# jerry102102102/RL_brain_trainer

Measured on NVIDIA B200. Metric: kinematic_env_steps_per_sec_policy_in_loop, higher is better.
Workload: dtype f32 env + f16 MLP operands (f32 accumulate)

## Files before the change

rl_brain_trainer_b200/csrc/kin_rollout_tc16.cu:

```cuda
#include <cstdlib>

#include "kin_tc16.cuh"

namespace kin {

using namespace tc16;

#ifdef KIN_TC16_TRACE
__device__ long long kin_tc16_trace_buf[8][16][12];
#define TC16_STAMP(slot) do { if (blockIdx.x == 0 && c.step_id >= 10 && c.step_id < 18 && (threadIdx.x & 31) == 0) \
        kin_tc16_trace_buf[c.step_id - 10][threadIdx.x >> 5][slot] = clock64(); } while (0)
#else
#define TC16_STAMP(slot)
#endif

struct Tile16 {
    unsigned char *X, *H;
    float* snap;
    unsigned x_lo, h_lo, w0_lo, w1_lo, wo_lo, wob_lo;
    unsigned mbar_saddr, cnt_saddr, full_saddr, tmem_d, tmem_row;
    unsigned x_row, h_row;
    volatile int* stamp;
    int row, n_warps;
    unsigned parity, arrivals;
    int step_id;
};

template <bool AT>
__device__ __forceinline__ void issue_layer16(int layer, unsigned tmem_d, unsigned x_lo, unsigned h_lo, unsigned w0_lo, unsigned w1_lo,
                                              unsigned wo_lo, unsigned wob_lo, unsigned mbar_saddr) {
    auto mma = [&](unsigned a, int ka, unsigned b_lo, unsigned id, unsigned acc) {
        if constexpr (AT) mma_f16_ts(tmem_d, a + 8u * ka, b_lo, id, acc);
        else mma_f16(tmem_d, a + 2u * ka, b_lo, id, acc);
    };
    if (layer == 0) {
        constexpr unsigned id = idesc_f16(TILE, HID);
#pragma unroll
        for (int k = 0; k < X_K / 16; ++k) mma(x_lo, k, w0_lo + 2 * k, id, k > 0 ? 1u : 0u);
    } else if (layer == 1) {
        constexpr unsigned id = idesc_f16(TILE, HID);
#pragma unroll
        for (int k = 0; k < HID / 16; ++k) mma(h_lo, k, w1_lo + 2 * k, id, k > 0 ? 1u : 0u);
        mma(x_lo, 2, w0_lo + 6, id, 1u);
    } else {
        constexpr unsigned id = idesc_f16(TILE, 16);
#pragma unroll
        for (int k = 0; k < HID / 16; ++k) mma(h_lo, k, wo_lo + 2 * k, id, k > 0 ? 1u : 0u);
        mma(x_lo, 2, wob_lo + 4, id, 1u);
    }
    umma::commit(mbar_saddr);
}

template <bool ISS, bool AT>
__device__ __forceinline__ void tile_sync16(Tile16& c, int layer, int sid) {
    TC16_STAMP(layer);
    if constexpr (AT) tmem_st_wait();
    if constexpr (ISS) {
        if constexpr (!AT) umma::fence_async_smem();
        umma::fence_before();
        __syncwarp();
        if ((threadIdx.x & 31) == 0) mbar_arrive(c.full_saddr);
    } else {
        c.arrivals += (unsigned)c.n_warps;
        if (const int last = tile_arrive(c.cnt_saddr, c.arrivals, layer == 0 ? c.stamp : nullptr, sid)) {
            umma::fence_after();
            if (elect_one()) {
                if (last == 1) issue_layer16<AT>(layer, c.tmem_d, c.x_lo, c.h_lo, c.w0_lo, c.w1_lo, c.wo_lo, c.wob_lo, c.mbar_saddr);
                else mbar_arrive(c.mbar_saddr);
            }
            __syncwarp();
            TC16_STAMP(6 + layer);
        }
    }
    mbar_wait_or_trap(c.mbar_saddr, c.parity);
    TC16_STAMP(3 + layer);
    c.parity ^= 1u;
}

template <bool ISS, bool AT>
__device__ __forceinline__ bool mlp16(Tile16& c, const unsigned* w, float* act, bool running) {
    const int sid = ++c.step_id;
    if (__any_sync(0xffffffffu, running) && (threadIdx.x & 31) == 0) *c.stamp = sid;
    if constexpr (AT) {
        tmem_st8(c.x_row, w);
        tmem_st8(c.x_row + 8u, w + 8);
        tmem_st4(c.x_row + 16u, w[16], w[17], 0x00003C00u, 0u);
    } else {
        st_chunk(c.X, c.row, 0, w[0], w[1], w[2], w[3]);
        st_chunk(c.X, c.row, 1, w[4], w[5], w[6], w[7]);
        st_chunk(c.X, c.row, 2, w[8], w[9], w[10], w[11]);
        st_chunk(c.X, c.row, 3, w[12], w[13], w[14], w[15]);
        st_chunk(c.X, c.row, 4, w[16], w[17], 0x00003C00u, 0u);
    }
    tile_sync16<ISS, AT>(c, 0, sid);
    if (*c.stamp != sid) return false;
    umma::fence_after();
    if constexpr (AT) epilogue_tanh_tmem(c.tmem_row, c.h_row);
    else epilogue_tanh(c.tmem_row, c.H, c.row);
    tile_sync16<ISS, AT>(c, 1, sid);
    umma::fence_after();
    if constexpr (AT) epilogue_tanh_tmem(c.tmem_row, c.h_row);
    else epilogue_tanh(c.tmem_row, c.H, c.row);
    tile_sync16<ISS, AT>(c, 2, sid);
    umma::fence_after();
    {
        float o[8];
        tmem_ld8(c.tmem_row, o);
#pragma unroll
        for (int i = 0; i < NJ; ++i) act[i] = clampf(o[i], -1.0f, 1.0f);
    }
    return true;
}

struct IssTile {
    unsigned x_lo, h_lo, tmem_d, full_saddr, mbar_saddr;
    volatile int* stamp;
    unsigned parity;
    int sid, layer, tile;
    bool exists, live;
};

template <bool AT>
__device__ __forceinline__ void issuer_poll(IssTile& t, unsigned w0_lo, unsigned w1_lo, unsigned wo_lo, unsigned wob_lo, unsigned hint_ns) {
    if (!(hint_ns ? mbar_try_wait_hint(t.full_saddr, t.parity, hint_ns) : mbar_test_wait(t.full_saddr, t.parity))) return;
    t.parity ^= 1u;
    umma::fence_after();
    bool go = true;
    if (t.layer == 0) {
        t.sid += 1;
        go = (*t.stamp == t.sid);
    }
#ifdef KIN_TC16_TRACE
    if (blockIdx.x == 0 && t.sid >= 10 && t.sid < 18 && (threadIdx.x & 31) == 0) kin_tc16_trace_buf[t.sid - 10][4 * t.tile][9 + t.layer] = clock64();
#endif
    if (elect_one()) {
        if (go) issue_layer16<AT>(t.layer, t.tmem_d, t.x_lo, t.h_lo, w0_lo, w1_lo, wo_lo, wob_lo, t.mbar_saddr);
        else mbar_arrive(t.mbar_saddr);
#ifdef KIN_TC16_TRACE
        if (blockIdx.x == 0 && t.sid >= 10 && t.sid < 18) kin_tc16_trace_buf[t.sid - 10][4 * t.tile][6 + t.layer] = clock64();
#endif
    }
    __syncwarp();
    if (!go) t.live = false;
    else t.layer = t.layer == 2 ? 0 : t.layer + 1;
}

__device__ unsigned kin_tc16_poll_hint = 32u;

template <bool AT>
__device__ __forceinline__ void issuer_phase(IssTile& a, IssTile& b, unsigned w0_lo, unsigned w1_lo, unsigned wo_lo, unsigned wob_lo) {
    a.live = a.exists;
    b.live = b.exists;
    a.layer = b.layer = 0;
    unsigned spins = 0u;
    while (a.live || b.live) {
        const unsigned hint = (a.live && b.live) ? kin_tc16_poll_hint : 1000u;
        if (a.live) issuer_poll<AT>(a, w0_lo, w1_lo, wo_lo, wob_lo, hint);
        if (b.live) issuer_poll<AT>(b, w0_lo, w1_lo, wo_lo, wob_lo, hint);
        if (++spins > (1u << 28)) __trap();
    }
}

__device__ __forceinline__ bool ready_pred16(float pos_thr, float ori_thr, float a_thr, float dq_thr, float pos, float ori, float an, float dqn) {
    return pos_thr > 0.0f && ori_thr > 0.0f && pos <= pos_thr && ori <= ori_thr && (a_thr <= 0.0f || an <= a_thr) && (dq_thr <= 0.0f || dqn <= dq_thr);
}

template <int FAST, bool ISS, bool AT>
__global__ void __launch_bounds__(MAX_THREADS, 1)
kin_rollout_tc16_kernel(const __grid_constant__ KinEnvParams PA, const __grid_constant__ KinEnvParams PF, DevPolicy pol_a, DevPolicy pol_f,
                        int has_finisher, const float* __restrict__ iq, const float* __restrict__ idq, const float* __restrict__ ipa,
                        const float* __restrict__ gq, const float* __restrict__ gpose, int n, int stride, int confirm,
                        uint32_t* __restrict__ result, unsigned long long* __restrict__ env_steps) {
    extern __shared__ __align__(1024) unsigned char smem_raw[];
    unsigned char* base = smem_raw + ((1024u - (umma::smem_u32(smem_raw) & 1023u)) & 1023u);
    Smem& S = *reinterpret_cast<Smem*>(base);
    const int tid = threadIdx.x;
    const int warp = tid >> 5;
    const int env_threads = (int)blockDim.x - (ISS ? 64 : 0);
    const int n_tiles_cta = (env_threads + TILE - 1) / TILE;
    unsigned char* tiles = base + ((sizeof(Smem) + 1023) / 1024) * 1024;
    float* snaps = reinterpret_cast<float*>(tiles + (size_t)n_tiles_cta * 2 * TILE_BYTES);

    Tile16 c;
    const int tile = tid >> 7;
    c.row = tid & (TILE - 1);
    c.n_warps = (min(TILE, env_threads - tile * TILE) + 31) >> 5;
    c.X = tiles + (size_t)tile * 2 * TILE_BYTES;
    c.H = c.X + TILE_BYTES;
    c.snap = snaps + (size_t)tile * SNAP_FLOATS * TILE + c.row;
    c.parity = 0u;
    c.arrivals = 0u;
    c.step_id = 0;
    c.stamp = &S.run_stamp[tile];

    constexpr unsigned TCOLS = AT ? 128u : 64u;
    const unsigned tmem_cols = n_tiles_cta == 1 ? TCOLS : (n_tiles_cta == 2 ? 2u * TCOLS : 4u * TCOLS);
    if (warp == 0) umma::tmem_alloc(umma::smem_u32(&S.tmem_base), tmem_cols);
    if (tid == 0) {
#pragma unroll
        for (int i = 0; i < MAX_TILES; ++i) {
            umma::mbar_init(umma::smem_u32(&S.mbar[i]), 1);
            umma::mbar_init(umma::smem_u32(&S.full[i]), (unsigned)max(1, (min(TILE, env_threads - i * TILE) + 31) >> 5));
            S.arrive[i] = 0u;
            S.run_stamp[i] = 0;
        }
        umma::fence_mbar_init();
    }
    load_weights(S, pol_a, KIN_MODE_APPROACH, tid, (int)blockDim.x);
    const bool env_thread = tid < env_threads;
    if (env_thread) {
#pragma unroll
        for (int ch = 0; ch < 8; ++ch) {
            st_chunk(c.X, c.row, ch, 0u, 0u, 0u, 0u);
            st_chunk(c.H, c.row, ch, 0u, 0u, 0u, 0u);
        }
    }
    if (env_thread && c.n_warps < 4) {
        for (int r = c.n_warps * 32 + c.row; r < TILE; r += c.n_warps * 32)
#pragma unroll
            for (int ch = 0; ch < 8; ++ch) {
                st_chunk(c.X, r, ch, 0u, 0u, 0u, 0u);
                st_chunk(c.H, r, ch, 0u, 0u, 0u, 0u);
            }
    }
    umma::fence_async_smem();
    umma::fence_before();
    __syncthreads();
    umma::fence_after();
    const unsigned tmem_base = S.tmem_base;
    c.x_lo = desc_lo(umma::smem_u32(c.X));
    c.h_lo = desc_lo(umma::smem_u32(c.H));
    c.w0_lo = desc_lo(umma::smem_u32(S.W0));
    c.w1_lo = desc_lo(umma::smem_u32(S.W1));
    c.wo_lo = desc_lo(umma::smem_u32(S.WO));
    c.wob_lo = desc_lo(umma::smem_u32(S.WOB));
    c.mbar_saddr = umma::smem_u32(&S.mbar[tile]);
    c.cnt_saddr = umma::smem_u32(&S.arrive[tile]);
    c.full_saddr = umma::smem_u32(&S.full[tile]);
    c.tmem_d = tmem_base + tile * TCOLS;
    c.tmem_row = c.tmem_d + ((unsigned)((warp & 3) * 32) << 16);
    c.h_row = c.tmem_row + 64u;
    c.x_row = c.tmem_row + 96u;
    if constexpr (AT) {
        c.x_lo = c.tmem_d + 96u;
        c.h_lo = c.tmem_d + 64u;
        if (env_thread) {
            tmem_st4(c.x_row + 20u, 0u, 0u, 0u, 0u);
            tmem_st4(c.x_row + 24u, 0u, 0u, 0u, 0u);
            tmem_st4(c.x_row + 28u, 0u, 0u, 0u, 0u);
            tmem_st_wait();
        }
    }

    if constexpr (ISS) {
        if (!env_thread) {
            const int iw = (tid - env_threads) >> 5;
            IssTile it[2];
#pragma unroll
            for (int j = 0; j < 2; ++j) {
                const int t = 2 * iw + j;
                it[j].exists = t < n_tiles_cta;
                it[j].tile = t;
                unsigned char* X = tiles + (size_t)t * 2 * TILE_BYTES;
                it[j].x_lo = desc_lo(umma::smem_u32(X));
                it[j].h_lo = desc_lo(umma::smem_u32(X + TILE_BYTES));
                it[j].tmem_d = tmem_base + t * TCOLS;
                if constexpr (AT) { it[j].x_lo = it[j].tmem_d + 96u; it[j].h_lo = it[j].tmem_d + 64u; }
                it[j].full_saddr = umma::smem_u32(&S.full[t]);
                it[j].mbar_saddr = umma::smem_u32(&S.mbar[t]);
                it[j].stamp = &S.run_stamp[t];
                it[j].parity = 0u;
                it[j].sid = 0;
            }
            issuer_phase<AT>(it[0], it[1], c.w0_lo, c.w1_lo, c.wo_lo, c.wob_lo);
            __syncthreads();
            if (has_finisher) {
                load_weights(S, pol_f, KIN_MODE_DOCK, tid, (int)blockDim.x);
                umma::fence_async_smem();
                __syncthreads();
                issuer_phase<AT>(it[0], it[1], c.w0_lo, c.w1_lo, c.wo_lo, c.wob_lo);
            }
            umma::fence_before();
            __syncthreads();
            return;
        }
    }

    const int ep = blockIdx.x * env_threads + tid;
    const bool active = ep < n;
    const int epc = active ? ep : n - 1;

    EnvRegs s;
    s.flags = 0u;
    float goal_q[NJ];
    {
        float r_iq[NJ], r_idq[NJ], r_ipa[NJ], r_gq[NJ], r_gp[6];
#pragma unroll
        for (int k = 0; k < NJ; ++k) {
            r_iq[k] = iq[(size_t)epc * NJ + k];
            r_idq[k] = idq ? idq[(size_t)epc * NJ + k] : 0.0f;
            r_ipa[k] = ipa ? ipa[(size_t)epc * NJ + k] : 0.0f;
            r_gq[k] = gq ? gq[(size_t)epc * NJ + k] : 0.0f;
        }
        if (gpose) {
#pragma unroll
            for (int k = 0; k < 6; ++k) r_gp[k] = gpose[(size_t)epc * 6 + k];
        }
        reset_core(PA, s, KIN_MODE_APPROACH, r_iq, r_idq, r_ipa, r_gq, gpose ? r_gp : nullptr, goal_q);
    }

    float min_pos = s.entry[0], min_ori = s.entry[1];
    int steps = 0, streak = 0, max_streak = 0, first_ready = -1;
    bool ready_hit = false, have_snap = false;
    int snap_step = -1;
    float last_an = 0.0f, last_dqn = 0.0f;
    StepOut so;
    prime_step_out(PA, s, so);
    bool running = active;
    while (true) {
        unsigned w[X_DYN / 2];
        float act[NJ];
        obs_pack(PA, s, so, w);
        if (!mlp16<ISS, AT>(c, w, act, running)) break;
        if (running) {
            step_core<KIN_MODE_APPROACH, false, FAST>(PA, s, act, so, nullptr);
            const float an = so.action_l2;
            steps += 1;
            min_pos = fminf(min_pos, so.pos);
            min_ori = fminf(min_ori, so.ori);
            if (ready_pred16(PA.ar_dock_coarse_ready_pos_threshold_m, PA.ar_dock_coarse_ready_ori_threshold_rad,
                             PA.ar_dock_coarse_ready_action_threshold, PA.ar_dock_coarse_ready_dq_threshold, so.pos, so.ori, an, so.dq_l2)) {
                ready_hit = true;
                if (first_ready < 0) first_ready = steps;
                streak += 1;
            } else {
                streak = 0;
            }
            max_streak = max(max_streak, streak);
            if (!have_snap && streak >= confirm) {
                have_snap = true;
                snap_step = steps;
#pragma unroll
                for (int i = 0; i < NJ; ++i) {
                    c.snap[i * TILE] = s.q[i];
                    c.snap[(NJ + i) * TILE] = s.dq[i];
                    c.snap[(2 * NJ + i) * TILE] = s.pa[i];
                }
            }
            last_an = an;
            last_dqn = so.dq_l2;
            running = !(so.done & (KIN_DONE_TERMINATED | KIN_DONE_TRUNCATED));
        }
    }
    if (active) {
        result[(size_t)KIN_RES_APPROACH_ACTION * stride + ep] = __float_as_uint(last_an);
        result[(size_t)KIN_RES_APPROACH_DQ * stride + ep] = __float_as_uint(last_dqn);
    }
    const int approach_steps = steps;
    const bool approach_success = (so.done & KIN_DONE_SUCCESS) != 0;
    const float approach_pos = so.pos, approach_ori = so.ori;
    const bool final_ready = ready_pred16(PA.ar_finisher_ready_pos_threshold_m, PA.ar_finisher_ready_ori_threshold_rad,
                                          PA.ar_finisher_ready_action_threshold, PA.ar_finisher_ready_dq_threshold, so.pos, so.ori, last_an, last_dqn);
    const int handoff_kind = final_ready ? 2 : (have_snap ? 1 : 0);
    const int handoff_step = final_ready ? steps : (have_snap ? snap_step : -1);
    bool success = approach_success;
    float final_pos = so.pos, final_ori = so.ori, final_an = last_an, final_dqn = last_dqn;
    int finisher_steps = 0;

    __syncthreads();
    if (has_finisher) {
        load_weights(S, pol_f, KIN_MODE_DOCK, tid, (int)blockDim.x);
        umma::fence_async_smem();
        __syncthreads();
        running = active && handoff_kind != 0;
        if (running) {
            float r_iq[NJ], r_idq[NJ], r_ipa[NJ], gq_out[NJ], r_gp[6];
#pragma unroll
            for (int i = 0; i < NJ; ++i) {
                r_iq[i] = (handoff_kind == 2) ? s.q[i] : c.snap[i * TILE];
                r_idq[i] = (handoff_kind == 2) ? s.dq[i] : c.snap[(NJ + i) * TILE];
                r_ipa[i] = (handoff_kind == 2) ? s.pa[i] : c.snap[(2 * NJ + i) * TILE];
            }
#pragma unroll
            for (int k = 0; k < 6; ++k) r_gp[k] = s.goal[k];
            reset_core(PF, s, KIN_MODE_DOCK, r_iq, r_idq, r_ipa, goal_q, r_gp, gq_out);
        }
        steps = 0;
        prime_step_out(PF, s, so);
        if (!running) { so.pos = final_pos; so.ori = final_ori; }
        while (true) {
            unsigned w[X_DYN / 2];
            float act[NJ];
            obs_pack(PF, s, so, w);
            if (!mlp16<ISS, AT>(c, w, act, running)) break;
            if (running) {
                float an2 = 0.0f;
#pragma unroll
                for (int i = 0; i < NJ; ++i) an2 = fmaf(act[i], act[i], an2);
                step_core<KIN_MODE_DOCK, false, FAST>(PF, s, act, so, nullptr);
                steps += 1;
                final_an = sqrt_approx(an2);
                running = !(so.done & (KIN_DONE_TERMINATED | KIN_DONE_TRUNCATED));
            }
        }
        if (active && handoff_kind != 0) {
            finisher_steps = steps;
            success = (so.done & KIN_DONE_SUCCESS) != 0;
            final_pos = so.pos; final_ori = so.ori; final_dqn = so.dq_l2;
        }
    }

    if (active) {
        auto put_u = [&](int row, uint32_t v) { result[(size_t)row * stride + ep] = v; };
        auto put_f = [&](int row, float v) { result[(size_t)row * stride + ep] = __float_as_uint(v); };
        put_u(KIN_RES_SUCCESS, success ? 1u : 0u);
        put_u(KIN_RES_FLAGS, (approach_success ? 1u : 0u) | ((ready_hit || final_ready) ? 2u : 0u) |
                                 ((max_streak >= confirm || final_ready) ? 4u : 0u) | (final_ready ? 8u : 0u) | ((uint32_t)handoff_kind << 4));
        put_u(KIN_RES_HANDOFF_STEP, (uint32_t)handoff_step);
        put_u(KIN_RES_FIRST_READY_STEP, (uint32_t)first_ready);
        put_u(KIN_RES_MAX_READY_STREAK, (uint32_t)max_streak);
        put_u(KIN_RES_STEPS, (uint32_t)approach_steps | ((uint32_t)finisher_steps << 16));
        put_f(KIN_RES_FINAL_POS, final_pos); put_f(KIN_RES_FINAL_ORI, final_ori);
        put_f(KIN_RES_APPROACH_POS, approach_pos); put_f(KIN_RES_APPROACH_ORI, approach_ori);
        put_f(KIN_RES_MIN_POS, min_pos); put_f(KIN_RES_MIN_ORI, min_ori);
        put_f(KIN_RES_FINAL_ACTION, final_an); put_f(KIN_RES_FINAL_DQ, final_dqn);
#pragma unroll
        for (int i = 0; i < NJ; ++i) put_f(KIN_RES_FINAL_Q + i, s.q[i]);
    }
    if (env_steps) {
        unsigned long long mine = active ? (unsigned long long)(approach_steps + finisher_steps) : 0ull;
#pragma unroll
        for (int off = 16; off > 0; off >>= 1) mine += __shfl_xor_sync(0xffffffffu, mine, off);
        if ((tid & 31) == 0 && mine) atomicAdd(env_steps, mine);
    }
    umma::fence_before();
    __syncthreads();
    if (warp == 0) umma::tmem_dealloc(tmem_base, tmem_cols);
}

}

using namespace kin;

#ifdef KIN_TC16_TRACE
extern "C" int kin_debug_tc16_trace(long long* out) {
    return cudaMemcpyFromSymbol(out, kin_tc16_trace_buf, sizeof(kin_tc16_trace_buf)) == cudaSuccess ? KIN_OK : KIN_ERR_INVALID_ARG;
}
#endif

int kin_rollout_tc16_launch(const KinHandle* ha, const KinHandle* hf, const KinPolicyWeights* pa, const KinPolicyWeights* pf,
                            const float* iq, const float* idq, const float* ipa, const float* gq, const float* gpose, int n, int stride,
                            int confirm, uint32_t* result, unsigned long long* env_steps, cudaStream_t st) {
    using Kernel = void (*)(KinEnvParams, KinEnvParams, tc16::DevPolicy, tc16::DevPolicy, int, const float*, const float*, const float*, const float*,
                            const float*, int, int, int, uint32_t*, unsigned long long*);
    static const Kernel kernels[2][2][2] = {{{kin_rollout_tc16_kernel<1, false, false>, kin_rollout_tc16_kernel<1, false, true>},
                                             {kin_rollout_tc16_kernel<1, true, false>, kin_rollout_tc16_kernel<1, true, true>}},
                                            {{kin_rollout_tc16_kernel<2, false, false>, kin_rollout_tc16_kernel<2, false, true>},
                                             {kin_rollout_tc16_kernel<2, true, false>, kin_rollout_tc16_kernel<2, true, true>}}};
    static bool attr_set[KIN_MAX_DEVICES] = {};
    const int dev_slot = kin_device_slot();
    if (!attr_set[dev_slot]) {
        for (int i = 0; i < 8; ++i) {
            cudaError_t e = cudaFuncSetAttribute(kernels[i >> 2][(i >> 1) & 1][i & 1], cudaFuncAttributeMaxDynamicSharedMemorySize, (int)tc16::smem_bytes(tc16::MAX_TILES));
            if (e != cudaSuccess) return kin_fail_cuda(e, "kin_rollout_approach_finisher(tc16): smem attribute");
        }
        attr_set[dev_slot] = true;
    }
    static const bool exact_sincos = kin_env_flag("KIN_TC16_EXACT_SINCOS");
    static const bool no_issuer = kin_env_flag("KIN_TC16_NO_ISSUER_WARPS");
    static const bool tmem_a = !kin_env_flag("KIN_TC16_SMEM_A");
    static bool hint_set = false;
    if (!hint_set) {
        if (const char* v = getenv("KIN_TC16_POLL_HINT")) { const unsigned h = (unsigned)atoi(v); cudaMemcpyToSymbol(kin_tc16_poll_hint, &h, sizeof(h)); }
        hint_set = true;
    }
    tc16::DevPolicy da{pa->pi_w0, pa->pi_b0, pa->pi_w1, pa->pi_b1, pa->act_w, pa->act_b};
    tc16::DevPolicy df = pf ? tc16::DevPolicy{pf->pi_w0, pf->pi_b0, pf->pi_w1, pf->pi_b1, pf->act_w, pf->act_b} : da;
    const KinEnvParams& PF = hf ? hf->params : ha->params;
    static int n_sm = 0;
    if (n_sm == 0) {
        int dev = 0;
        if (cudaGetDevice(&dev) != cudaSuccess || cudaDeviceGetAttribute(&n_sm, cudaDevAttrMultiProcessorCount, dev) != cudaSuccess || n_sm <= 0) n_sm = 148;
    }
    const int warps = (n + 31) / 32;
    int w_per_cta = (warps + n_sm - 1) / n_sm;
    if (w_per_cta > 16) w_per_cta = 16;
    if (const char* v = getenv("KIN_TC_WARPS")) { const int f = atoi(v); if (f >= 1 && f <= 16) w_per_cta = f; }
    const bool iss = w_per_cta <= 14 && !no_issuer;
    const int env_threads = 32 * w_per_cta;
    const int threads = env_threads + (iss ? 64 : 0);
    const size_t smem = tc16::smem_bytes((env_threads + tc16::TILE - 1) / tc16::TILE);
    kernels[exact_sincos ? 0 : 1][iss ? 1 : 0][tmem_a ? 1 : 0]<<<(n + env_threads - 1) / env_threads, threads, smem, st>>>(
        ha->params, PF, da, df, (hf && pf) ? 1 : 0, iq, idq, ipa, gq, gpose, n, stride, confirm, result, env_steps);
    cudaError_t e = cudaGetLastError();
    return e == cudaSuccess ? KIN_OK : kin_fail_cuda(e, "kin_rollout_approach_finisher(tc16)");
}
```

rl_brain_trainer_b200/csrc/kin_tc16.cuh:

```cuda
#pragma once

#include <cuda_fp16.h>

#include "kin_internal.h"
#include "kin_state.cuh"
#include "kin_umma.cuh"

namespace kin {
namespace tc16 {

using namespace umma;

constexpr int TILE = 128;
constexpr int MAX_TILES = 4;
constexpr int MAX_THREADS = TILE * MAX_TILES;
constexpr int HID = 64;
constexpr int X_DYN = 36;
constexpr int X_ONE = 36;
constexpr int X_K = 48;
constexpr int B1_COL = 52;
constexpr int TILE_BYTES = TILE * 128;
constexpr int SNAP_FLOATS = 3 * KIN_NJ;

struct Smem {
    alignas(1024) unsigned char W0[HID * 128];
    alignas(1024) unsigned char W1[HID * 128];
    alignas(1024) unsigned char WO[16 * 128];
    alignas(1024) unsigned char WOB[16 * 128];
    unsigned long long mbar[MAX_TILES];
    unsigned long long full[MAX_TILES];
    unsigned arrive[MAX_TILES];
    int run_stamp[MAX_TILES];
    unsigned tmem_base;
};

struct DevPolicy {
    const float *w0, *b0, *w1, *b1, *wo, *bo;
};

__host__ __device__ constexpr size_t smem_bytes(int n_tiles) {
    return ((sizeof(Smem) + 1023) / 1024) * 1024 + (size_t)n_tiles * (2 * TILE_BYTES + SNAP_FLOATS * TILE * sizeof(float)) + 1024;
}

__host__ __device__ constexpr unsigned idesc_f16(int M, int N) { return (1u << 4) | ((unsigned)(N >> 3) << 17) | ((unsigned)(M >> 4) << 24); }

__device__ __forceinline__ unsigned pack_h2(float lo, float hi) {
    unsigned r;
    asm("cvt.rn.f16x2.f32 %0, %1, %2;" : "=r"(r) : "f"(hi), "f"(lo));
    return r;
}
__device__ __forceinline__ unsigned clamp1_h2(unsigned x) {
    unsigned y;
    asm("{\n\t.reg .b32 t;\n\tmax.f16x2 t, %1, %2;\n\tmin.f16x2 %0, t, %3;\n\t}" : "=r"(y) : "r"(x), "r"(0xBC00BC00u), "r"(0x3C003C00u));
    return y;
}
__device__ __forceinline__ void st_chunk(unsigned char* img, int row, int chunk, unsigned a, unsigned b, unsigned c, unsigned d) {
    *reinterpret_cast<uint4*>(img + umma::sw_chunk(row, chunk)) = make_uint4(a, b, c, d);
}

__device__ __forceinline__ int dyn_col(int k) { return k < 20 ? k : (k < 27 ? k + 10 : (k < 29 ? k + 10 : k + 11)); }

__device__ __forceinline__ void obs_pack(const KinEnvParams& P, const EnvRegs& s, const StepOut& so, unsigned* w) {
    float v[X_DYN];
#pragma unroll
    for (int i = 0; i < NJ; ++i) {
        v[i] = s.dq[i] * P.k_inv_delta_limit[i];
        v[13 + i] = so.margin[i];
        v[20 + i] = s.pa[i];
        v[29 + i] = so.qn[i];
    }
#pragma unroll
    for (int k = 0; k < 3; ++k) {
        v[7 + k] = so.oe[k] * P.k_inv_ori_err_scale;
        v[10 + k] = so.pe[k] * P.k_inv_pos_err_scale;
    }
    v[27] = (float)s.step * P.k_inv_episode_length;
    v[28] = (float)s.dwell * P.k_inv_dwell_steps_target;
#pragma unroll
    for (int i = 0; i < X_DYN / 2; ++i) w[i] = pack_h2(v[2 * i], v[2 * i + 1]);
#pragma unroll
    for (int i = 0; i < X_DYN / 2; ++i)
        if (!((i >= 7 && i <= 9) || i >= 15)) w[i] = clamp1_h2(w[i]);
}

__device__ __forceinline__ void prime_step_out(const KinEnvParams& P, const EnvRegs& s, StepOut& so) {
    so.done = 0u;
    so.pos = s.entry[0];
    so.ori = s.entry[1];
    so.dq_l2 = 0.0f;
    pose_error(s.ee, s.goal, so.pe, so.oe);
#pragma unroll
    for (int i = 0; i < NJ; ++i) {
        so.qn[i] = qnorm(P, s.q[i], i);
        so.margin[i] = 1.0f - fabsf(so.qn[i]);
    }
}

__device__ __forceinline__ void load_weights(Smem& S, const DevPolicy& p, int mode, int tid, int nthreads) {
    for (int i = tid; i < HID * 64; i += nthreads) {
        const int n = i >> 6, k = i & 63;
        float v0 = 0.0f;
        if (k < X_DYN) v0 = __ldg(p.w0 + n * KIN_OBS_DIM + dyn_col(k));
        else if (k == X_ONE) v0 = __ldg(p.b0 + n) + __ldg(p.w0 + n * KIN_OBS_DIM + 20 + mode) + __ldg(p.w0 + n * KIN_OBS_DIM + 47);
        else if (k == B1_COL) v0 = __ldg(p.b1 + n);
        *reinterpret_cast<__half*>(S.W0 + umma::sw_elem(n, k)) = __float2half_rn(v0);
        *reinterpret_cast<__half*>(S.W1 + umma::sw_elem(n, k)) = __float2half_rn(__ldg(p.w1 + n * HID + k));
    }
    for (int i = tid; i < 16 * 64; i += nthreads) {
        const int n = i >> 6, k = i & 63;
        *reinterpret_cast<__half*>(S.WO + umma::sw_elem(n, k)) = __float2half_rn(n < KIN_NJ ? __ldg(p.wo + n * HID + k) : 0.0f);
        *reinterpret_cast<__half*>(S.WOB + umma::sw_elem(n, k)) = __float2half_rn((n < KIN_NJ && k == X_ONE) ? __ldg(p.bo + n) : 0.0f);
    }
}

constexpr unsigned DESC_HI = 64u | (1u << 14) | (2u << 29);
__device__ __forceinline__ unsigned desc_lo(unsigned saddr) { return ((saddr >> 4) & 0x3FFFu) | (1u << 16); }
__device__ __forceinline__ void mma_f16(unsigned tmem_d, unsigned a_lo, unsigned b_lo, unsigned idesc, unsigned accumulate) {
    asm volatile(
        "{\n\t.reg .pred p;\n\t.reg .b64 da, db;\n\t"
        "setp.ne.b32 p, %4, 0;\n\t"
        "mov.b64 da, {%1, %5};\n\t"
        "mov.b64 db, {%2, %5};\n\t"
        "tcgen05.mma.cta_group::1.kind::f16 [%0], da, db, %3, p;\n\t}"
        ::"r"(tmem_d), "r"(a_lo), "r"(b_lo), "r"(idesc), "r"(accumulate), "r"(DESC_HI) : "memory");
}
__device__ __forceinline__ void mma_f16_ts(unsigned tmem_d, unsigned a_taddr, unsigned b_lo, unsigned idesc, unsigned accumulate) {
    asm volatile(
        "{\n\t.reg .pred p;\n\t.reg .b64 db;\n\t"
        "setp.ne.b32 p, %4, 0;\n\t"
        "mov.b64 db, {%2, %5};\n\t"
        "tcgen05.mma.cta_group::1.kind::f16 [%0], [%1], db, %3, p;\n\t}"
        ::"r"(tmem_d), "r"(a_taddr), "r"(b_lo), "r"(idesc), "r"(accumulate), "r"(DESC_HI) : "memory");
}
__device__ __forceinline__ int tile_arrive(unsigned cnt_saddr, unsigned target, const volatile int* stamp = nullptr, int sid = 0) {
    umma::fence_async_smem();
    umma::fence_before();
    __syncwarp();
    int last = 0;
    if ((threadIdx.x & 31) == 0) {
        unsigned old;
        asm volatile("atom.relaxed.cta.shared::cta.add.u32 %0, [%1], 1;" : "=r"(old) : "r"(cnt_saddr) : "memory");
        if (old + 1u == target) last = (stamp == nullptr || *stamp == sid) ? 1 : 2;
    }
    return __shfl_sync(0xffffffffu, last, 0);
}

__device__ __forceinline__ void tanh_store16(const unsigned* r, unsigned char* H, int row, int ch2) {
#pragma unroll
    for (int h = 0; h < 2; ++h) {
        unsigned w[4];
#pragma unroll
        for (int j = 0; j < 4; ++j)
            w[j] = pack_h2(umma::tanh_fast(__uint_as_float(r[8 * h + 2 * j])), umma::tanh_fast(__uint_as_float(r[8 * h + 2 * j + 1])));
        st_chunk(H, row, 2 * ch2 + h, w[0], w[1], w[2], w[3]);
    }
}

__device__ __forceinline__ void tanh_store16_tmem(const unsigned* r, unsigned h_taddr, int piece) {
    unsigned w[8];
#pragma unroll
    for (int j = 0; j < 8; ++j) w[j] = pack_h2(umma::tanh_fast(__uint_as_float(r[2 * j])), umma::tanh_fast(__uint_as_float(r[2 * j + 1])));
    tmem_st8(h_taddr + 8u * piece, w);
}
__device__ __forceinline__ void epilogue_tanh_tmem(unsigned tmem_row, unsigned h_taddr) {
    unsigned a[16], b[16];
    tmem_ld16_raw(tmem_row, a);
    tmem_wait16(a);
    tmem_ld16_raw(tmem_row + 16u, b);
    tanh_store16_tmem(a, h_taddr, 0);
    tmem_wait16(b);
    tmem_ld16_raw(tmem_row + 32u, a);
    tanh_store16_tmem(b, h_taddr, 1);
    tmem_wait16(a);
    tmem_ld16_raw(tmem_row + 48u, b);
    tanh_store16_tmem(a, h_taddr, 2);
    tmem_wait16(b);
    tanh_store16_tmem(b, h_taddr, 3);
}

__device__ __forceinline__ void epilogue_tanh(unsigned tmem_row, unsigned char* H, int row) {
    unsigned a[16], b[16];
    tmem_ld16_raw(tmem_row, a);
    tmem_wait16(a);
    tmem_ld16_raw(tmem_row + 16u, b);
    tanh_store16(a, H, row, 0);
    tmem_wait16(b);
    tmem_ld16_raw(tmem_row + 32u, a);
    tanh_store16(b, H, row, 1);
    tmem_wait16(a);
    tmem_ld16_raw(tmem_row + 48u, b);
    tanh_store16(a, H, row, 2);
    tmem_wait16(b);
    tanh_store16(b, H, row, 3);
}

}
}
```

Before: 16.16 billion.

## Preload both policy weight images to remove mid-kernel barrier and reload

Shared memory now holds two weight images, one per policy. Both the approach and finisher policies are loaded at kernel start, so the CTA-wide __syncthreads and the weight reload between the approach and finisher phases go away. Each tile switches policy by offsetting its descriptor, and the issuer warp moves a tile to finisher weights on its own when that tile stops, so tiles no longer wait for the slowest tile in the CTA. The cost is a larger shared-memory footprint for weights; to offset it, the TMEM-A variant drops the now-unused X/H shared buffers and the epilogue code is unified.

```diff
diff --git a/rl_brain_trainer_b200/csrc/kin_rollout_tc16.cu b/rl_brain_trainer_b200/csrc/kin_rollout_tc16.cu
--- a/rl_brain_trainer_b200/csrc/kin_rollout_tc16.cu
+++ b/rl_brain_trainer_b200/csrc/kin_rollout_tc16.cu
@@ -17,7 +17,7 @@
 struct Tile16 {
     unsigned char *X, *H;
     float* snap;
-    unsigned x_lo, h_lo, w0_lo, w1_lo, wo_lo, wob_lo;
+    unsigned x_lo, h_lo, w_lo;
     unsigned mbar_saddr, cnt_saddr, full_saddr, tmem_d, tmem_row;
     unsigned x_row, h_row;
     volatile int* stamp;
@@ -27,8 +27,7 @@
 };
 
 template <bool AT>
-__device__ __forceinline__ void issue_layer16(int layer, unsigned tmem_d, unsigned x_lo, unsigned h_lo, unsigned w0_lo, unsigned w1_lo,
-                                              unsigned wo_lo, unsigned wob_lo, unsigned mbar_saddr) {
+__device__ __forceinline__ void issue_layer16(int layer, unsigned tmem_d, unsigned x_lo, unsigned h_lo, unsigned w_lo, unsigned mbar_saddr) {
     auto mma = [&](unsigned a, int ka, unsigned b_lo, unsigned id, unsigned acc) {
         if constexpr (AT) mma_f16_ts(tmem_d, a + 8u * ka, b_lo, id, acc);
         else mma_f16(tmem_d, a + 2u * ka, b_lo, id, acc);
@@ -36,17 +35,17 @@
     if (layer == 0) {
         constexpr unsigned id = idesc_f16(TILE, HID);
 #pragma unroll
-        for (int k = 0; k < X_K / 16; ++k) mma(x_lo, k, w0_lo + 2 * k, id, k > 0 ? 1u : 0u);
+        for (int k = 0; k < X_K / 16; ++k) mma(x_lo, k, w_lo + 2 * k, id, k > 0 ? 1u : 0u);
     } else if (layer == 1) {
         constexpr unsigned id = idesc_f16(TILE, HID);
 #pragma unroll
-        for (int k = 0; k < HID / 16; ++k) mma(h_lo, k, w1_lo + 2 * k, id, k > 0 ? 1u : 0u);
-        mma(x_lo, 2, w0_lo + 6, id, 1u);
+        for (int k = 0; k < HID / 16; ++k) mma(h_lo, k, w_lo + W1_DESC + 2 * k, id, k > 0 ? 1u : 0u);
+        mma(x_lo, 2, w_lo + 6, id, 1u);
     } else {
         constexpr unsigned id = idesc_f16(TILE, 16);
 #pragma unroll
-        for (int k = 0; k < HID / 16; ++k) mma(h_lo, k, wo_lo + 2 * k, id, k > 0 ? 1u : 0u);
-        mma(x_lo, 2, wob_lo + 4, id, 1u);
+        for (int k = 0; k < HID / 16; ++k) mma(h_lo, k, w_lo + WO_DESC + 2 * k, id, k > 0 ? 1u : 0u);
+        mma(x_lo, 2, w_lo + WOB_DESC + 4, id, 1u);
     }
     umma::commit(mbar_saddr);
 }
@@ -65,7 +64,7 @@
         if (const int last = tile_arrive(c.cnt_saddr, c.arrivals, layer == 0 ? c.stamp : nullptr, sid)) {
             umma::fence_after();
             if (elect_one()) {
-                if (last == 1) issue_layer16<AT>(layer, c.tmem_d, c.x_lo, c.h_lo, c.w0_lo, c.w1_lo, c.wo_lo, c.wob_lo, c.mbar_saddr);
+                if (last == 1) issue_layer16<AT>(layer, c.tmem_d, c.x_lo, c.h_lo, c.w_lo, c.mbar_saddr);
                 else mbar_arrive(c.mbar_saddr);
             }
             __syncwarp();
@@ -75,6 +74,37 @@
     mbar_wait_or_trap(c.mbar_saddr, c.parity);
     TC16_STAMP(3 + layer);
     c.parity ^= 1u;
+}
+
+template <bool AT>
+__device__ __forceinline__ void store_h8(const Tile16& c, const unsigned* w, int piece) {
+    if constexpr (AT) {
+        tmem_st8(c.h_row + 8u * piece, w);
+    } else {
+        st_chunk(c.H, c.row, 2 * piece, w[0], w[1], w[2], w[3]);
+        st_chunk(c.H, c.row, 2 * piece + 1, w[4], w[5], w[6], w[7]);
+    }
+}
+
+template <bool AT>
+__device__ __forceinline__ void epilogue16(const Tile16& c) {
+    unsigned a[16], b[16], h[8];
+    tmem_ld16_raw(c.tmem_row, a);
+    tmem_wait16(a);
+    tmem_ld16_raw(c.tmem_row + 16u, b);
+    tanh_pack16(a, h);
+    store_h8<AT>(c, h, 0);
+    tmem_wait16(b);
+    tmem_ld16_raw(c.tmem_row + 32u, a);
+    tanh_pack16(b, h);
+    store_h8<AT>(c, h, 1);
+    tmem_wait16(a);
+    tmem_ld16_raw(c.tmem_row + 48u, b);
+    tanh_pack16(a, h);
+    store_h8<AT>(c, h, 2);
+    tmem_wait16(b);
+    tanh_pack16(b, h);
+    store_h8<AT>(c, h, 3);
 }
 
 template <bool ISS, bool AT>
@@ -95,12 +125,10 @@
     tile_sync16<ISS, AT>(c, 0, sid);
     if (*c.stamp != sid) return false;
     umma::fence_after();
-    if constexpr (AT) epilogue_tanh_tmem(c.tmem_row, c.h_row);
-    else epilogue_tanh(c.tmem_row, c.H, c.row);
+    epilogue16<AT>(c);
     tile_sync16<ISS, AT>(c, 1, sid);
     umma::fence_after();
-    if constexpr (AT) epilogue_tanh_tmem(c.tmem_row, c.h_row);
-    else epilogue_tanh(c.tmem_row, c.H, c.row);
+    epilogue16<AT>(c);
     tile_sync16<ISS, AT>(c, 2, sid);
     umma::fence_after();
     {
@@ -113,15 +141,15 @@
 }
 
 struct IssTile {
-    unsigned x_lo, h_lo, tmem_d, full_saddr, mbar_saddr;
+    unsigned x_lo, h_lo, w_lo, tmem_d, full_saddr, mbar_saddr;
     volatile int* stamp;
     unsigned parity;
     int sid, layer, tile;
-    bool exists, live;
+    bool live, finisher;
 };
 
 template <bool AT>
-__device__ __forceinline__ void issuer_poll(IssTile& t, unsigned w0_lo, unsigned w1_lo, unsigned wo_lo, unsigned wob_lo, unsigned hint_ns) {
+__device__ __forceinline__ void issuer_poll(IssTile& t, bool has_finisher, unsigned hint_ns) {
     if (!(hint_ns ? mbar_try_wait_hint(t.full_saddr, t.parity, hint_ns) : mbar_test_wait(t.full_saddr, t.parity))) return;
     t.parity ^= 1u;
     umma::fence_after();
@@ -134,29 +162,32 @@
     if (blockIdx.x == 0 && t.sid >= 10 && t.sid < 18 && (threadIdx.x & 31) == 0) kin_tc16_trace_buf[t.sid - 10][4 * t.tile][9 + t.layer] = clock64();
 #endif
     if (elect_one()) {
-        if (go) issue_layer16<AT>(t.layer, t.tmem_d, t.x_lo, t.h_lo, w0_lo, w1_lo, wo_lo, wob_lo, t.mbar_saddr);
+        if (go) issue_layer16<AT>(t.layer, t.tmem_d, t.x_lo, t.h_lo, t.w_lo, t.mbar_saddr);
         else mbar_arrive(t.mbar_saddr);
 #ifdef KIN_TC16_TRACE
         if (blockIdx.x == 0 && t.sid >= 10 && t.sid < 18) kin_tc16_trace_buf[t.sid - 10][4 * t.tile][6 + t.layer] = clock64();
 #endif
     }
     __syncwarp();
-    if (!go) t.live = false;
-    else t.layer = t.layer == 2 ? 0 : t.layer + 1;
+    if (go) {
+        t.layer = t.layer == 2 ? 0 : t.layer + 1;
+    } else if (has_finisher && !t.finisher) {
+        t.finisher = true;
+        t.w_lo += POL_DESC;
+    } else {
+        t.live = false;
+    }
 }
 
 __device__ unsigned kin_tc16_poll_hint = 32u;
 
 template <bool AT>
-__device__ __forceinline__ void issuer_phase(IssTile& a, IssTile& b, unsigned w0_lo, unsigned w1_lo, unsigned wo_lo, unsigned wob_lo) {
-    a.live = a.exists;
-    b.live = b.exists;
-    a.layer = b.layer = 0;
+__device__ __forceinline__ void issuer_loop(IssTile& a, IssTile& b, bool has_finisher) {
     unsigned spins = 0u;
     while (a.live || b.live) {
         const unsigned hint = (a.live && b.live) ? kin_tc16_poll_hint : 1000u;
-        if (a.live) issuer_poll<AT>(a, w0_lo, w1_lo, wo_lo, wob_lo, hint);
-        if (b.live) issuer_poll<AT>(b, w0_lo, w1_lo, wo_lo, wob_lo, hint);
+        if (a.live) issuer_poll<AT>(a, has_finisher, hint);
+        if (b.live) issuer_poll<AT>(b, has_finisher, hint);
         if (++spins > (1u << 28)) __trap();
     }
 }
@@ -179,7 +210,7 @@
     const int env_threads = (int)blockDim.x - (ISS ? 64 : 0);
     const int n_tiles_cta = (env_threads + TILE - 1) / TILE;
     unsigned char* tiles = base + ((sizeof(Smem) + 1023) / 1024) * 1024;
-    float* snaps = reinterpret_cast<float*>(tiles + (size_t)n_tiles_cta * 2 * TILE_BYTES);
+    float* snaps = reinterpret_cast<float*>(tiles + (AT ? 0 : (size_t)n_tiles_cta * 2 * TILE_BYTES));
 
     Tile16 c;
     const int tile = tid >> 7;
@@ -206,22 +237,25 @@
         }
         umma::fence_mbar_init();
     }
-    load_weights(S, pol_a, KIN_MODE_APPROACH, tid, (int)blockDim.x);
+    load_weights(S.pol[0], pol_a, KIN_MODE_APPROACH, tid, (int)blockDim.x);
+    if (has_finisher) load_weights(S.pol[1], pol_f, KIN_MODE_DOCK, tid, (int)blockDim.x);
     const bool env_thread = tid < env_threads;
-    if (env_thread) {
-#pragma unroll
-        for (int ch = 0; ch < 8; ++ch) {
-            st_chunk(c.X, c.row, ch, 0u, 0u, 0u, 0u);
-            st_chunk(c.H, c.row, ch, 0u, 0u, 0u, 0u);
-        }
-    }
-    if (env_thread && c.n_warps < 4) {
-        for (int r = c.n_warps * 32 + c.row; r < TILE; r += c.n_warps * 32)
+    if constexpr (!AT) {
+        if (env_thread) {
 #pragma unroll
             for (int ch = 0; ch < 8; ++ch) {
-                st_chunk(c.X, r, ch, 0u, 0u, 0u, 0u);
-                st_chunk(c.H, r, ch, 0u, 0u, 0u, 0u);
-            }
+                st_chunk(c.X, c.row, ch, 0u, 0u, 0u, 0u);
+                st_chunk(c.H, c.row, ch, 0u, 0u, 0u, 0u);
+            }
+        }
+        if (env_thread && c.n_warps < 4) {
+            for (int r = c.n_warps * 32 + c.row; r < TILE; r += c.n_warps * 32)
+#pragma unroll
+                for (int ch = 0; ch < 8; ++ch) {
+                    st_chunk(c.X, r, ch, 0u, 0u, 0u, 0u);
+                    st_chunk(c.H, r, ch, 0u, 0u, 0u, 0u);
+                }
+        }
     }
     umma::fence_async_smem();
     umma::fence_before();
@@ -230,10 +264,7 @@
     const unsigned tmem_base = S.tmem_base;
     c.x_lo = desc_lo(umma::smem_u32(c.X));
     c.h_lo = desc_lo(umma::smem_u32(c.H));
-    c.w0_lo = desc_lo(umma::smem_u32(S.W0));
-    c.w1_lo = desc_lo(umma::smem_u32(S.W1));
-    c.wo_lo = desc_lo(umma::smem_u32(S.WO));
-    c.wob_lo = desc_lo(umma::smem_u32(S.WOB));
+    c.w_lo = desc_lo(umma::smem_u32(S.pol[0].W0));
     c.mbar_saddr = umma::smem_u32(&S.mbar[tile]);
     c.cnt_saddr = umma::smem_u32(&S.arrive[tile]);
     c.full_saddr = umma::smem_u32(&S.full[tile]);
@@ -259,7 +290,8 @@
 #pragma unroll
             for (int j = 0; j < 2; ++j) {
                 const int t = 2 * iw + j;
-                it[j].exists = t < n_tiles_cta;
+                it[j].live = t < n_tiles_cta;
+                it[j].finisher = false;
                 it[j].tile = t;
                 unsigned char* X = tiles + (size_t)t * 2 * TILE_BYTES;
                 it[j].x_lo = desc_lo(umma::smem_u32(X));
@@ -268,18 +300,13 @@
                 if constexpr (AT) { it[j].x_lo = it[j].tmem_d + 96u; it[j].h_lo = it[j].tmem_d + 64u; }
                 it[j].full_saddr = umma::smem_u32(&S.full[t]);
                 it[j].mbar_saddr = umma::smem_u32(&S.mbar[t]);
+                it[j].w_lo = c.w_lo;
                 it[j].stamp = &S.run_stamp[t];
                 it[j].parity = 0u;
                 it[j].sid = 0;
-            }
-            issuer_phase<AT>(it[0], it[1], c.w0_lo, c.w1_lo, c.wo_lo, c.wob_lo);
-            __syncthreads();
-            if (has_finisher) {
-                load_weights(S, pol_f, KIN_MODE_DOCK, tid, (int)blockDim.x);
-                umma::fence_async_smem();
-                __syncthreads();
-                issuer_phase<AT>(it[0], it[1], c.w0_lo, c.w1_lo, c.wo_lo, c.wob_lo);
-            }
+                it[j].layer = 0;
+            }
+            issuer_loop<AT>(it[0], it[1], has_finisher != 0);
             umma::fence_before();
             __syncthreads();
             return;
@@ -367,11 +394,8 @@
     float final_pos = so.pos, final_ori = so.ori, final_an = last_an, final_dqn = last_dqn;
     int finisher_steps = 0;
 
-    __syncthreads();
     if (has_finisher) {
-        load_weights(S, pol_f, KIN_MODE_DOCK, tid, (int)blockDim.x);
-        umma::fence_async_smem();
-        __syncthreads();
+        c.w_lo += POL_DESC;
         running = active && handoff_kind != 0;
         if (running) {
             float r_iq[NJ], r_idq[NJ], r_ipa[NJ], gq_out[NJ], r_gp[6];
@@ -461,7 +485,8 @@
     const int dev_slot = kin_device_slot();
     if (!attr_set[dev_slot]) {
         for (int i = 0; i < 8; ++i) {
-            cudaError_t e = cudaFuncSetAttribute(kernels[i >> 2][(i >> 1) & 1][i & 1], cudaFuncAttributeMaxDynamicSharedMemorySize, (int)tc16::smem_bytes(tc16::MAX_TILES));
+            cudaError_t e = cudaFuncSetAttribute(kernels[i >> 2][(i >> 1) & 1][i & 1], cudaFuncAttributeMaxDynamicSharedMemorySize,
+                                                 (int)tc16::smem_bytes(tc16::MAX_TILES, (i & 1) != 0));
             if (e != cudaSuccess) return kin_fail_cuda(e, "kin_rollout_approach_finisher(tc16): smem attribute");
         }
         attr_set[dev_slot] = true;
@@ -489,7 +514,7 @@
     const bool iss = w_per_cta <= 14 && !no_issuer;
     const int env_threads = 32 * w_per_cta;
     const int threads = env_threads + (iss ? 64 : 0);
-    const size_t smem = tc16::smem_bytes((env_threads + tc16::TILE - 1) / tc16::TILE);
+    const size_t smem = tc16::smem_bytes((env_threads + tc16::TILE - 1) / tc16::TILE, tmem_a);
     kernels[exact_sincos ? 0 : 1][iss ? 1 : 0][tmem_a ? 1 : 0]<<<(n + env_threads - 1) / env_threads, threads, smem, st>>>(
         ha->params, PF, da, df, (hf && pf) ? 1 : 0, iq, idq, ipa, gq, gpose, n, stride, confirm, result, env_steps);
     cudaError_t e = cudaGetLastError();
diff --git a/rl_brain_trainer_b200/csrc/kin_tc16.cuh b/rl_brain_trainer_b200/csrc/kin_tc16.cuh
--- a/rl_brain_trainer_b200/csrc/kin_tc16.cuh
+++ b/rl_brain_trainer_b200/csrc/kin_tc16.cuh
@@ -1,6 +1,8 @@
 #pragma once
 
 #include <cuda_fp16.h>
+
+#include <cstddef>
 
 #include "kin_internal.h"
 #include "kin_state.cuh"
@@ -22,11 +24,15 @@
 constexpr int TILE_BYTES = TILE * 128;
 constexpr int SNAP_FLOATS = 3 * KIN_NJ;
 
-struct Smem {
+struct WeightImg {
     alignas(1024) unsigned char W0[HID * 128];
     alignas(1024) unsigned char W1[HID * 128];
     alignas(1024) unsigned char WO[16 * 128];
     alignas(1024) unsigned char WOB[16 * 128];
+};
+
+struct Smem {
+    WeightImg pol[2];
     unsigned long long mbar[MAX_TILES];
     unsigned long long full[MAX_TILES];
     unsigned arrive[MAX_TILES];
@@ -38,8 +44,8 @@
     const float *w0, *b0, *w1, *b1, *wo, *bo;
 };
 
-__host__ __device__ constexpr size_t smem_bytes(int n_tiles) {
-    return ((sizeof(Smem) + 1023) / 1024) * 1024 + (size_t)n_tiles * (2 * TILE_BYTES + SNAP_FLOATS * TILE * sizeof(float)) + 1024;
+__host__ __device__ constexpr size_t smem_bytes(int n_tiles, bool at) {
+    return ((sizeof(Smem) + 1023) / 1024) * 1024 + (size_t)n_tiles * ((at ? 0 : 2 * TILE_BYTES) + SNAP_FLOATS * TILE * sizeof(float)) + 1024;
 }
 
 __host__ __device__ constexpr unsigned idesc_f16(int M, int N) { return (1u << 4) | ((unsigned)(N >> 3) << 17) | ((unsigned)(M >> 4) << 24); }
@@ -96,7 +102,7 @@
     }
 }
 
-__device__ __forceinline__ void load_weights(Smem& S, const DevPolicy& p, int mode, int tid, int nthreads) {
+__device__ __forceinline__ void load_weights(WeightImg& S, const DevPolicy& p, int mode, int tid, int nthreads) {
     for (int i = tid; i < HID * 64; i += nthreads) {
         const int n = i >> 6, k = i & 63;
         float v0 = 0.0f;
@@ -115,6 +121,8 @@
 
 constexpr unsigned DESC_HI = 64u | (1u << 14) | (2u << 29);
 __device__ __forceinline__ unsigned desc_lo(unsigned saddr) { return ((saddr >> 4) & 0x3FFFu) | (1u << 16); }
+constexpr unsigned W1_DESC = offsetof(WeightImg, W1) >> 4, WO_DESC = offsetof(WeightImg, WO) >> 4, WOB_DESC = offsetof(WeightImg, WOB) >> 4;
+constexpr unsigned POL_DESC = sizeof(WeightImg) >> 4;
 __device__ __forceinline__ void mma_f16(unsigned tmem_d, unsigned a_lo, unsigned b_lo, unsigned idesc, unsigned accumulate) {
     asm volatile(
         "{\n\t.reg .pred p;\n\t.reg .b64 da, db;\n\t"
@@ -145,53 +153,9 @@
     return __shfl_sync(0xffffffffu, last, 0);
 }
 
-__device__ __forceinline__ void tanh_store16(const unsigned* r, unsigned char* H, int row, int ch2) {
-#pragma unroll
-    for (int h = 0; h < 2; ++h) {
-        unsigned w[4];
-#pragma unroll
-        for (int j = 0; j < 4; ++j)
-            w[j] = pack_h2(umma::tanh_fast(__uint_as_float(r[8 * h + 2 * j])), umma::tanh_fast(__uint_as_float(r[8 * h + 2 * j + 1])));
-        st_chunk(H, row, 2 * ch2 + h, w[0], w[1], w[2], w[3]);
-    }
-}
-
-__device__ __forceinline__ void tanh_store16_tmem(const unsigned* r, unsigned h_taddr, int piece) {
-    unsigned w[8];
+__device__ __forceinline__ void tanh_pack16(const unsigned* r, unsigned* w) {
 #pragma unroll
     for (int j = 0; j < 8; ++j) w[j] = pack_h2(umma::tanh_fast(__uint_as_float(r[2 * j])), umma::tanh_fast(__uint_as_float(r[2 * j + 1])));
-    tmem_st8(h_taddr + 8u * piece, w);
-}
-__device__ __forceinline__ void epilogue_tanh_tmem(unsigned tmem_row, unsigned h_taddr) {
-    unsigned a[16], b[16];
-    tmem_ld16_raw(tmem_row, a);
-    tmem_wait16(a);
-    tmem_ld16_raw(tmem_row + 16u, b);
-    tanh_store16_tmem(a, h_taddr, 0);
-    tmem_wait16(b);
-    tmem_ld16_raw(tmem_row + 32u, a);
-    tanh_store16_tmem(b, h_taddr, 1);
-    tmem_wait16(a);
-    tmem_ld16_raw(tmem_row + 48u, b);
-    tanh_store16_tmem(a, h_taddr, 2);
-    tmem_wait16(b);
-    tanh_store16_tmem(b, h_taddr, 3);
-}
-
-__device__ __forceinline__ void epilogue_tanh(unsigned tmem_row, unsigned char* H, int row) {
-    unsigned a[16], b[16];
-    tmem_ld16_raw(tmem_row, a);
-    tmem_wait16(a);
-    tmem_ld16_raw(tmem_row + 16u, b);
-    tanh_store16(a, H, row, 0);
-    tmem_wait16(b);
-    tmem_ld16_raw(tmem_row + 32u, a);
-    tanh_store16(b, H, row, 1);
-    tmem_wait16(a);
-    tmem_ld16_raw(tmem_row + 48u, b);
-    tanh_store16(a, H, row, 2);
-    tmem_wait16(b);
-    tanh_store16(b, H, row, 3);
 }
 
 }
```

Result: no change. 16.24 billion, median of 6 (+0.5%).
